# Parskatt/RoMa

Hardware: NVIDIA H100
Metric: image-pairs/sec match()+sample() 560->864 (higher is better)
Workload: dtype f32 (activations f32; GEMM operands as split-f16 pairs hi + 2^-11 lo on wgmma, f32 accumulate: fp32-class)

## Files before the change

### include/romab200.h

```cpp
#ifndef ROMAB200_H
#define ROMAB200_H

#include <stdint.h>

#ifdef __cplusplus
extern "C" {
#endif

#define ROMAB200_ABI_VERSION 4

enum rb_dtype { RB_F32 = 0, RB_F16 = 1, RB_BF16 = 2, RB_F16S = 3, RB_F64 = 4 };
enum rb_act { RB_ACT_NONE = 0, RB_ACT_RELU = 1, RB_ACT_GELU = 2 };
enum rb_rowmap { RB_ROWMAP_NONE = 0, RB_ROWMAP_PAD_KEEP = 1, RB_ROWMAP_PAD_TO_COMPACT = 2, RB_ROWMAP_SEGMENT = 3 };
enum rb_epi { RB_EPI_LINEAR = 0, RB_EPI_COSKERNEL = 1 };
enum rb_backend { RB_BACKEND_AUTO = 0, RB_BACKEND_SIMT = 1, RB_BACKEND_TCGEN05 = 2 };

int romab200_abi_version(void);
const char* romab200_last_error(void);
unsigned long long romab200_launch_count(void);
int romab200_device_ok(void);

typedef struct {
    const void* A; const void* B; void* C;
    int32_t M, N, K;
    int64_t lda, ldb, ldc;
    int32_t dtype_ab, dtype_c;
    int32_t trans_b;
    int32_t batch0, batch1;
    int64_t sa0, sa1, sb0, sb1, sc0, sc1;
    int32_t ntaps; int32_t tap_rows[9]; int64_t a_rows;
    float alpha;
    const float* bias; const float* col_scale;
    const void* R; int64_t ldr, sr0, sr1; int32_t dtype_r;
    int32_t act;
    int32_t epi;
    const float* norm_a; const float* norm_b; int64_t sna0, snb0;
    float eps, inv_t, diag_add; int32_t cos_normalized;
    int32_t rowmap, pad_h, pad_w, seg_in, seg_out, seg_off;
    int32_t backend;
    const void* A_lo; const void* B_lo; void* C_lo;
    int32_t max_ctas;
} rb_gemm_args;
int romab200_gemm(const rb_gemm_args* args, void* stream);

typedef struct {
    const void* x; void* y; const float* gamma; const float* beta;
    int64_t rows; int32_t cols; int64_t ldx, ldy; int32_t dtype_x, dtype_y; float eps;
    void* y_lo;
} rb_layernorm_args;
int romab200_layernorm(const rb_layernorm_args* args, void* stream);

typedef struct { void* s; int64_t rows; int32_t cols; int64_t lds; int32_t dtype; float scale;
                 void* out_hi; void* out_lo; int64_t ldo; } rb_softmax_args;
int romab200_softmax_rows(const rb_softmax_args* args, void* stream);

typedef struct {
    const void* qkv; void* out; int64_t ld_qkv, ld_out; int32_t batch, n_tokens, heads, head_dim, dtype;
    const void* qkv_lo; void* out_lo;
} rb_flash_attn_args;
int romab200_flash_attn(const rb_flash_attn_args* args, void* stream);

typedef struct { const void* x; float* out; int64_t rows; int32_t cols; int64_t ldx; int32_t dtype; } rb_rownorm_args;
int romab200_row_norms(const rb_rownorm_args* args, void* stream);

typedef struct {
    const void* src; void* dst; int64_t rows; int32_t cols; int64_t lds, ldd; int32_t dtype_src, dtype_dst;
    const float* row_scale; int32_t row_scale_reciprocal;
} rb_copy2d_args;
int romab200_copy2d(const rb_copy2d_args* args, void* stream);

typedef struct {
    const void* src; void* dst; const int32_t* src_index; const int32_t* dst_index;
    int32_t count; int64_t row_bytes, ld_src, ld_dst; int32_t src_rows, dst_rows;
} rb_gather_rows_args;
int romab200_gather_rows(const rb_gather_rows_args* args, void* stream);

typedef struct {
    const float* x; void* dst; int64_t rows; int32_t cols; int64_t ldx, ldd; const float* row_norm;
    int32_t layout_b;
} rb_split_args;
int romab200_split_f16x3(const rb_split_args* args, void* stream);

typedef struct {
    const float* x; void* hi; void* lo; int64_t rows; int32_t cols; int64_t ldx, ldd; const float* row_norm;
} rb_split_pair_args;
int romab200_split_f16s(const rb_split_pair_args* args, void* stream);

typedef struct {
    const float* image; void* out; const float* weight ; const float* bias ;
    int32_t batch, height, width, cout; int32_t dtype_out;
    void* out_lo;
} rb_conv_first_args;
int romab200_conv3x3_first(const rb_conv_first_args* args, void* stream);
typedef struct { const void* in; void* out; int32_t batch, height, width, channels, dtype;
                 const void* in_lo; void* out_lo;  } rb_maxpool_args;
int romab200_maxpool2x2_padded(const rb_maxpool_args* args, void* stream);

typedef struct { const float* image; void* out; int32_t batch, height, width, patch; int64_t ldo; int32_t dtype_out; } rb_im2col_args;
int romab200_im2col_patch(const rb_im2col_args* args, void* stream);
typedef struct { const float* patch; const float* cls; const float* pos; float* tokens; int32_t batch, npatch, dim; } rb_tokens_args;
int romab200_assemble_tokens(const rb_tokens_args* args, void* stream);

typedef struct {
    float* W; int32_t n, nrhs, batch; int64_t ldw, stride;
    void* workspace; int64_t workspace_bytes;
    int32_t algo;
} rb_gp_solve_args;
int romab200_gp_solve(const rb_gp_solve_args* args, void* stream);
typedef struct { const void* logits; float* state; int64_t rows; int64_t ldl; int32_t res; int32_t dtype; } rb_cls_args;
int romab200_cls_to_flow_refine(const rb_cls_args* args, void* stream);

typedef struct {
    const void* feat; int64_t ldf; int32_t n_img, y_shift;
    const float* state; void* d; int64_t ldd;
    int32_t D, h, w, cf, emb, radius; int32_t dtype;
    const float* emb_weight ; const float* emb_bias; float disp_scale;
    const float* grid_x; const float* grid_y;
    const float* win_x; const float* win_y;
    void* tile_done; int32_t tile_done_len;
    const float* corr_table; int64_t ld_corr_table;
} rb_refiner_prologue_args;
int romab200_refiner_prologue(const rb_refiner_prologue_args* args, void* stream);

typedef struct {
    const void* f0; const void* f1; int64_t ldf0, ldf1; int64_t f0_img_stride, f1_img_stride;
    const float* flow; int64_t ldflow; void* out; int64_t ldo;
    int32_t batch, h, w, c, radius; float scale; int32_t dtype_f, dtype_out;
    int32_t n_img, y_shift;
    const float* win_x; const float* win_y;
} rb_local_corr_args;
int romab200_local_corr(const rb_local_corr_args* args, void* stream);

typedef struct {
    const float* f0; const float* f1; int64_t ldf0, ldf1; const float* warp; float* out;
    int32_t batch, h, w, c, k; int32_t mode;
} rb_local_corr_warp_args;
int romab200_local_corr_warp(const rb_local_corr_warp_args* args, void* stream);

typedef struct {
    const void* in; void* out; int64_t ldi, ldo; const float* weight; int64_t ldw; const float* bias;
    int32_t batch, h, w, c; int32_t dtype;
    void* out_lo;
} rb_dwconv_args;
int romab200_dwconv5x5_relu(const rb_dwconv_args* args, void* stream);

typedef struct {
    const void* in; void* out; int64_t ld; const float* dw_weight; int64_t ldw; const float* dw_bias;
    const float* pw_weight_host; const float* pw_bias_host; int32_t batch, h, w, c; int32_t dtype;
} rb_refiner_block_small_args;
int romab200_refiner_block_small(const rb_refiner_block_small_args* args, void* stream);

typedef struct {
    const void* in; void* out; int64_t ld; const float* dw_weight; int64_t ldw; const float* dw_bias;
    const void* pw_weight; int64_t ld_pw; const float* pw_bias; int32_t batch, h, w, c; int32_t dtype;
} rb_refiner_block_c144_args;
int romab200_refiner_block_c144(const rb_refiner_block_c144_args* args, void* stream);

typedef struct {
    const float* in; float* out; int64_t ld; const float* dw_weight; int64_t ldw; const float* dw_bias;
    const void* pw_weight; const void* pw_weight_lo; int64_t ld_pw; const float* pw_bias; int32_t batch, h, w, c;
} rb_refiner_block_c144_split_args;
int romab200_refiner_block_c144_split(const rb_refiner_block_c144_split_args* args, void* stream);

typedef struct {
    const void* d; int64_t ldd; const float* weight ; int64_t ldw; const float* bias;
    float* state; int64_t rows; int32_t c; float scale_x, scale_y; int32_t dtype; float* delta_out ;
} rb_refiner_tail_args;
int romab200_refiner_tail(const rb_refiner_tail_args* args, void* stream);

typedef struct { const float* in; float* out; int32_t batch, hi, wi, ho, wo, c; } rb_resize_args;
int romab200_bilinear_resize(const rb_resize_args* args, void* stream);

typedef struct {
    const float* state; const float* coarse_state; int32_t hc, wc;
    float* warp; float* cert; int32_t b, H, W, symmetric;
    const float* grid_x; const float* grid_y;
} rb_match_epilogue_args;
int romab200_match_epilogue(const rb_match_epilogue_args* args, void* stream);

typedef struct { const float* x; float* density; int32_t n; float std; int32_t half;
                 float* workspace; int32_t splits;
                 int32_t symmetric; int64_t workspace_floats;
                 int32_t batch; } rb_kde_args;
int romab200_kde_density(const rb_kde_args* args, void* stream);

enum rb_sample_transform { RB_SAMPLE_IDENTITY = 0, RB_SAMPLE_THRESHOLD = 1, RB_SAMPLE_BALANCE = 2 };
typedef struct {
    const float* values; int64_t n; int32_t k; int32_t batch; int64_t stride; uint64_t seed; int32_t transform; float param;
    int32_t* out_idx; float* out_weights; float* keys;
    void* scratch;
    const uint64_t* seed_dev;
    int64_t seed_stride; int32_t repeats;
} rb_sample_args;
int romab200_weighted_sample(const rb_sample_args* args, void* stream);

typedef struct {
    const float* matches; const float* certainty; int64_t n;
    const int32_t* idx; int32_t items, k, repeats;
    int32_t threshold; float thresh;
    float* out_matches; float* out_certainty;
} rb_sample_gather_args;
int romab200_sample_gather(const rb_sample_gather_args* args, void* stream);

typedef struct { int32_t in_size, out_size; int32_t* bounds; int32_t* kk; int32_t* ksize; } rb_resample_coeffs_args;
int romab200_resample_coeffs(const rb_resample_coeffs_args* args, void* stream);

typedef struct {
    const uint8_t* in; int64_t ld_in ; int32_t in_h, in_w;
    int32_t out_h, out_w;
    const int32_t* bounds_x; const int32_t* kk_x; int32_t ksize_x;
    const int32_t* bounds_y; const int32_t* kk_y; int32_t ksize_y;
    uint8_t* tmp;
    uint8_t* out_u8;
    float* out;
    float mean[3]; float std[3];
} rb_preprocess_args;
int romab200_preprocess_rgb8(const rb_preprocess_args* args, void* stream);

typedef struct {
    const void* src; void* dst; int32_t rows, cols; int64_t lds, ldd; int32_t batch0, batch1;
    int64_t ss0, ss1, sd0, sd1; int32_t dtype;
} rb_transpose_args;
int romab200_transpose(const rb_transpose_args* args, void* stream);

typedef struct {
    const float* x; int32_t n;
    const float* warp; int32_t warp_h, warp_w; int64_t warp_ld_row, warp_ld_px, warp_ld_ch;
    const float* cert; int32_t cert_h, cert_w; int64_t cert_ld_row, cert_ld_px;
    float* x_to_B; float* cert_out;
} rb_keypoints_sample_args;
int romab200_keypoints_sample(const rb_keypoints_sample_args* args, void* stream);

typedef struct {
    const float* x_A_to_B; const float* cert_A; const float* x_B; int32_t n_a, n_b;
    float cert_th, max_dist;
    float* workspace; int64_t workspace_floats;
    int64_t* offsets;
    int64_t* inds_A; int64_t* inds_B;
} rb_keypoints_mnn_args;
int romab200_keypoints_mnn_count(const rb_keypoints_mnn_args* args, void* stream);
int romab200_keypoints_mnn_emit(const rb_keypoints_mnn_args* args, void* stream);

typedef struct {
    const float* in; float* out; const float* weight; const float* bias; const float* col_scale; const float* R;
    int64_t ldi, ldo, ldw, ldr;
    int32_t batch, hi, wi, ho, wo, cin, cout, ksize, stride, relu;
} rb_tiny_conv_args;
int romab200_tiny_conv(const rb_tiny_conv_args* args, void* stream);

typedef struct { const float* in; float* out; int32_t batch, channels, h, w, instance_norm; float eps; } rb_tiny_gray_args;
int romab200_tiny_gray(const rb_tiny_gray_args* args, void* stream);

typedef struct { const float* in; float* out; int32_t batch, hi, wi, c; } rb_tiny_avgpool_args;
int romab200_tiny_avgpool4(const rb_tiny_avgpool_args* args, void* stream);

typedef struct { const float* a; const float* b; const float* c; float* out; int64_t n; } rb_tiny_add3_args;
int romab200_tiny_add3(const rb_tiny_add3_args* args, void* stream);

typedef struct {
    const float* f0; const float* f1; float* state;
    int32_t batch, h0, w0, h1, w1, c; float scale; int32_t exact;
    const float* grid_x; const float* grid_y; const float* grid_lr_x; const float* grid_lr_y;
} rb_tiny_pos_embed_args;
int romab200_tiny_pos_embed(const rb_tiny_pos_embed_args* args, void* stream);

typedef struct {
    const float* f0; const float* f1; const float* state; float* out;
    int64_t ldf0, ldf1, lds, ldo; int32_t batch, h0, w0, h1, w1, c;
} rb_tiny_warp_concat_args;
int romab200_tiny_warp_concat(const rb_tiny_warp_concat_args* args, void* stream);

typedef struct { const float* state; float* warp; float* cert; int32_t batch, h, w; const float* grid_x; const float* grid_y; } rb_tiny_epilogue_args;
int romab200_tiny_match_epilogue(const rb_tiny_epilogue_args* args, void* stream);

typedef struct {
    int32_t batch;
    const uint8_t* stream;
    const int64_t* desc;
    const int32_t* tables;
    uint8_t* comp;
    int32_t* chunks;
    int32_t* istart;
    int64_t* exits;
    int32_t* counts;
    int16_t* coef;
    int32_t* state;
    int32_t* flags;
    int32_t max_chunks, max_intervals;
    int64_t total_slots, total_blocks;
    uint8_t* planes;
    uint8_t* out;
    int64_t max_pixels;
} rb_jpeg_args;
int romab200_jpeg_entropy(const rb_jpeg_args* args, void* stream);
int romab200_jpeg_pixels(const rb_jpeg_args* args, void* stream);

#define RB_POSE_ROUND 1024
#define RB_POSE_MAX_SOL 10
#define RB_POSE_MAX_SPLITS 16
#define RB_POSE_STATE 8
typedef struct {
    int32_t batch;
    const double* x0; const double* x1;
    const int64_t* offsets;
    const double* K;
    int64_t max_n;
    double thresh, conf;
    int32_t max_iters, round;
    uint64_t seed;
    double* xn;
    int32_t* sample;
    double* E;
    int32_t* nsol;
    int32_t* counts;
    int32_t* state;
    double* best_E;
    int32_t* running;
    double* R; double* t;
    uint8_t* ok;
    uint8_t* mask;
} rb_pose_args;
int romab200_pose_hypotheses(const rb_pose_args* args, void* stream);
int romab200_pose_score(const rb_pose_args* args, void* stream);
int romab200_pose_select(const rb_pose_args* args, void* stream);
int romab200_pose_recover(const rb_pose_args* args, void* stream);

#define RB_HOMOG_ROUND 2048
#define RB_HOMOG_MAX_SPLITS 32
#define RB_HOMOG_MAX_ATTEMPTS 10000
#define RB_HOMOG_STATE 8
typedef struct {
    int32_t batch;
    const float* src; const float* dst;
    const int64_t* offsets;
    int64_t max_n;
    double thresh, conf;
    int32_t max_iters, round, method;
    uint64_t seed;
    int32_t* sample;
    int32_t* attempts;
    int32_t* status;
    double* H;
    int32_t* counts;
    int32_t* state;
// ... 328 lines not shown
```

### roma_b200/csrc/gemm_tc.cu

```cuda
#include "tma.cuh"
#include "wgmma.cuh"

namespace rb {

struct TcParams {
    int M, N, K;
    int batch1;
    int ntaps, k_per_tap; int tap_rows[9];
    int tiles_m, tiles_n, total_tiles;
    int band_m;
    int n_zero_to;
    int64_t sc0, sc1, sr0, sr1, sna0, snb0;
    Epilogue epi;
};

constexpr int TC_BM = 128, TC_BK = 64;
constexpr int TC_THREADS = 384;
constexpr int TC_CW = 32, TC_SP = 40;
constexpr int TC_STAGING = 2 * 64 * TC_SP * 4;

template <int BN, bool SPLIT> struct TcCfg {
    static constexpr int NOPS = SPLIT ? 2 : 1;
    static constexpr int A_BYTES = TC_BM * TC_BK * 2;
    static constexpr int B_BYTES = BN * TC_BK * 2;
    static constexpr int STAGE_BYTES = NOPS * (A_BYTES + B_BYTES);
    static constexpr int RING_MAX = 232448 - TC_STAGING - 1024  - 256 ;
    static constexpr int STAGES = RING_MAX / STAGE_BYTES > 8 ? 8 : RING_MAX / STAGE_BYTES;
    static constexpr int SMEM = STAGES * STAGE_BYTES + TC_STAGING + 1024 + 256;
    static_assert(STAGES >= 3 && SMEM <= 232448, "shared memory budget");
};

__device__ __forceinline__ void load8(const void* p, int64_t i, int dtype, int cnt, float (&v)[8]) {
    if (dtype == RB_F32) {
        const float* s = (const float*)p + i;
        if (cnt == 8 && (reinterpret_cast<uintptr_t>(s) & 15) == 0) {
            const float4 a = reinterpret_cast<const float4*>(s)[0], b = reinterpret_cast<const float4*>(s)[1];
            v[0] = a.x; v[1] = a.y; v[2] = a.z; v[3] = a.w; v[4] = b.x; v[5] = b.y; v[6] = b.z; v[7] = b.w;
        } else {
#pragma unroll
            for (int k = 0; k < 8; ++k) v[k] = k < cnt ? s[k] : 0.f;
        }
        return;
    }
    const uint16_t* s = (const uint16_t*)p + i;
    uint16_t h[8];
    if (cnt == 8 && (reinterpret_cast<uintptr_t>(s) & 15) == 0) {
        const uint4 q = *reinterpret_cast<const uint4*>(s);
        const uint32_t w[4] = {q.x, q.y, q.z, q.w};
#pragma unroll
        for (int k = 0; k < 4; ++k) { h[2 * k] = (uint16_t)w[k]; h[2 * k + 1] = (uint16_t)(w[k] >> 16); }
    } else {
#pragma unroll
        for (int k = 0; k < 8; ++k) h[k] = k < cnt ? s[k] : 0;
    }
    if (dtype == RB_F16) {
#pragma unroll
        for (int k = 0; k < 8; ++k) v[k] = __half2float(__ushort_as_half(h[k]));
    } else {
#pragma unroll
        for (int k = 0; k < 8; ++k) v[k] = __bfloat162float(__ushort_as_bfloat16(h[k]));
    }
}

__device__ __forceinline__ void store8(const Epilogue& e, int64_t i, int cnt, const float (&v)[8]) {
    if (e.dtype_c == RB_F32) {
        float* c = (float*)e.C + i;
        if (cnt == 8 && (reinterpret_cast<uintptr_t>(c) & 15) == 0) {
            reinterpret_cast<float4*>(c)[0] = make_float4(v[0], v[1], v[2], v[3]);
            reinterpret_cast<float4*>(c)[1] = make_float4(v[4], v[5], v[6], v[7]);
        } else {
#pragma unroll
            for (int k = 0; k < 8; ++k) if (k < cnt) c[k] = v[k];
        }
        return;
    }
    uint16_t h[8], l[8];
    const bool two = e.dtype_c == RB_F16S;
    if (e.dtype_c == RB_BF16) {
#pragma unroll
        for (int k = 0; k < 8; ++k) h[k] = __bfloat16_as_ushort(__float2bfloat16_rn(v[k]));
    } else {
#pragma unroll
        for (int k = 0; k < 8; ++k) {
            __half hi, lo;
            split_f16s(v[k], hi, lo);
            h[k] = __half_as_ushort(hi); l[k] = __half_as_ushort(lo);
        }
    }
    uint16_t* c = (uint16_t*)e.C + i;
    uint16_t* cl = two ? (uint16_t*)e.C_lo + i : nullptr;
    if (cnt == 8 && (reinterpret_cast<uintptr_t>(c) & 15) == 0 && (!two || (reinterpret_cast<uintptr_t>(cl) & 15) == 0)) {
        *reinterpret_cast<uint4*>(c) = make_uint4(h[0] | (uint32_t)h[1] << 16, h[2] | (uint32_t)h[3] << 16, h[4] | (uint32_t)h[5] << 16,
                                                  h[6] | (uint32_t)h[7] << 16);
        if (two) *reinterpret_cast<uint4*>(cl) = make_uint4(l[0] | (uint32_t)l[1] << 16, l[2] | (uint32_t)l[3] << 16,
                                                            l[4] | (uint32_t)l[5] << 16, l[6] | (uint32_t)l[7] << 16);
    } else {
#pragma unroll
        for (int k = 0; k < 8; ++k) if (k < cnt) { c[k] = h[k]; if (two) cl[k] = l[k]; }
    }
}

__device__ __forceinline__ void epilogue8(const Epilogue& e, int m, int n, int64_t orow, int cnt, const float (&cb)[8],
                                          const float (&cs)[8], float na, float (&v)[8]) {
    const int nv = min(8, e.N - n);
    if (e.epi == RB_EPI_COSKERNEL) {
#pragma unroll
        for (int k = 0; k < 8; ++k) {
            const float p = na * cb[k];
            const float s = e.cos_normalized ? p / (p + e.eps) : 1.0f / (p + e.eps);
            v[k] = expf((v[k] * s - 1.0f) * e.inv_t);
            if (m == n + k) v[k] += e.diag_add;
        }
    } else {
#pragma unroll
        for (int k = 0; k < 8; ++k) v[k] = __fmul_rn(e.alpha, v[k]);
        if (e.bias) {
#pragma unroll
            for (int k = 0; k < 8; ++k) v[k] = __fadd_rn(v[k], cb[k]);
        }
        if (e.act == RB_ACT_RELU) {
#pragma unroll
            for (int k = 0; k < 8; ++k) v[k] = fmaxf(v[k], 0.0f);
        } else if (e.act == RB_ACT_GELU) {
#pragma unroll
            for (int k = 0; k < 8; ++k) v[k] = gelu_erf(v[k]);
        }
        if (e.col_scale) {
#pragma unroll
            for (int k = 0; k < 8; ++k) v[k] = __fmul_rn(v[k], cs[k]);
        }
        if (e.R) {
            float r[8];
            load8(e.R, orow * e.ldr + n, e.dtype_r, nv, r);
#pragma unroll
            for (int k = 0; k < 8; ++k) v[k] = __fadd_rn(v[k], r[k]);
        }
    }
    if (nv < 8) {
#pragma unroll
        for (int k = 0; k < 8; ++k) if (k >= nv) v[k] = 0.f;
    }
    store8(e, orow * e.ldc + n, cnt, v);
}

__device__ __forceinline__ void tile_coords(const TcParams& p, int w, int& z, int& mt, int& nt) {
    const int per_z = p.tiles_m * p.tiles_n;
    z = w / per_z;
    const int r = w - z * per_z;
    const int m_lo = r / (p.band_m * p.tiles_n) * p.band_m;
    const int rows = min(p.band_m, p.tiles_m - m_lo);
    const int rb = r - m_lo * p.tiles_n;
    nt = rb / rows;
    mt = m_lo + (rb - nt * rows);
}

template <int BN, bool SPLIT, bool BF16, int TB>
__global__ void __launch_bounds__(TC_THREADS, 1)
gemm_tc_kernel(const __grid_constant__ CUtensorMap map_a, const __grid_constant__ CUtensorMap map_b,
               const __grid_constant__ CUtensorMap map_a_lo, const __grid_constant__ CUtensorMap map_b_lo, const TcParams p) {
    using Cfg = TcCfg<BN, SPLIT>;
    constexpr int STAGES = Cfg::STAGES;
    constexpr int A_BYTES = Cfg::A_BYTES, B_BYTES = Cfg::B_BYTES;
    constexpr int OFF_A_LO = A_BYTES, OFF_B = Cfg::NOPS * A_BYTES, OFF_B_LO = Cfg::NOPS * A_BYTES + B_BYTES;
    extern __shared__ uint8_t smem_raw[];
    uint8_t* smem = smem_raw + ((1024u - ((uint32_t)__cvta_generic_to_shared(smem_raw) & 1023u)) & 1023u);
    float* staging = reinterpret_cast<float*>(smem + STAGES * Cfg::STAGE_BYTES);
    uint64_t* full_bar = reinterpret_cast<uint64_t*>(smem + STAGES * Cfg::STAGE_BYTES + TC_STAGING);
    uint64_t* empty_bar = full_bar + STAGES;

    const int warp = threadIdx.x >> 5, lane = threadIdx.x & 31;
    const int kblocks = (p.K + TC_BK - 1) / TC_BK;

    if (threadIdx.x == 0) {
        for (int s = 0; s < STAGES; ++s) { mbar_init(&full_bar[s], 1); mbar_init(&empty_bar[s], 2); }
        asm volatile("fence.mbarrier_init.release.cluster;" ::: "memory");
    }
    __syncthreads();
    rb::pdl_wait();

    if (warp >= 8) {
        asm volatile("setmaxnreg.dec.sync.aligned.u32 40;");
        if (warp == 8 && lane == 0) {
            const int kb_per_tap = p.ntaps > 1 ? p.k_per_tap / TC_BK : kblocks;
            uint32_t it = 0;
            for (int tile = blockIdx.x; tile < p.total_tiles; tile += gridDim.x) {
                int z, mt, nt;
                tile_coords(p, tile, z, mt, nt);
                const int m0 = mt * TC_BM, n0 = nt * BN, z0 = z / p.batch1, z1 = z - z0 * p.batch1;
                for (int kb = 0; kb < kblocks; ++kb, ++it) {
                    const int s = it % STAGES;
                    const uint32_t ph = (it / STAGES) & 1;
                    mbar_wait(&empty_bar[s], ph ^ 1);
                    mbar_expect_tx(&full_bar[s], Cfg::STAGE_BYTES);
                    int tap = 0, kin = kb * TC_BK, shift = 0;
                    if (p.ntaps > 1) { tap = kb / kb_per_tap; kin = (kb - tap * kb_per_tap) * TC_BK; shift = p.tap_rows[tap]; }
                    uint8_t* st = smem + s * Cfg::STAGE_BYTES;
                    tma_load_4d(st, &map_a, &full_bar[s], kin, m0 + shift, z1, z0);
                    if constexpr (SPLIT) tma_load_4d(st + OFF_A_LO, &map_a_lo, &full_bar[s], kin, m0 + shift, z1, z0);
                    if constexpr (!TB) {
                        tma_load_4d(st + OFF_B, &map_b, &full_bar[s], kb * TC_BK, n0, z1, z0);
                        if constexpr (SPLIT) tma_load_4d(st + OFF_B_LO, &map_b_lo, &full_bar[s], kb * TC_BK, n0, z1, z0);
                    } else {
#pragma unroll
                        for (int j = 0; j < (BN + 63) / 64; ++j) {
                            tma_load_4d(st + OFF_B + j * (64 * 128), &map_b, &full_bar[s], n0 + j * 64, kb * TC_BK, z1, z0);
                            if constexpr (SPLIT) tma_load_4d(st + OFF_B_LO + j * (64 * 128), &map_b_lo, &full_bar[s], n0 + j * 64, kb * TC_BK, z1, z0);
                        }
                    }
                }
            }
        }
        return;
    }

    asm volatile("setmaxnreg.inc.sync.aligned.u32 232;");
    const int wg = warp >> 2, t = threadIdx.x & 127;
    float acc[BN / 2];
    float acc2[SPLIT ? BN / 2 : 1];
    uint32_t it = 0;
    for (int tile = blockIdx.x; tile < p.total_tiles; tile += gridDim.x) {
        int z, mt, nt;
        tile_coords(p, tile, z, mt, nt);
        const int m0 = mt * TC_BM, n0 = nt * BN, z0 = z / p.batch1, z1 = z - z0 * p.batch1;
        int prev = -1;
        for (int kb = 0; kb < kblocks; ++kb, ++it) {
            const int s = it % STAGES;
            mbar_wait(&full_bar[s], (it / STAGES) & 1);
            const uint32_t st = smem_u32(smem + s * Cfg::STAGE_BYTES);
            wgmma_fence();
#pragma unroll
            for (int k = 0; k < TC_BK / 16; ++k) {
                const uint32_t koff_a = wg * (64 * 128) + k * 32;
                const uint32_t koff_b = TB ? k * 2048 : k * 32;
                const uint32_t lbo_b = TB ? 64 * 128 : 16;
                const uint64_t a_hi = gmma_desc(st + koff_a, 16, 1024);
                const uint64_t b_hi = gmma_desc(st + OFF_B + koff_b, lbo_b, 1024);
                const int accum = (kb | k) != 0;
                Wgmma<BN, BF16>::template ss<TB>(acc, a_hi, b_hi, accum);
                if constexpr (SPLIT) {
                    const uint64_t a_lo = gmma_desc(st + OFF_A_LO + koff_a, 16, 1024);
                    const uint64_t b_lo = gmma_desc(st + OFF_B_LO + koff_b, lbo_b, 1024);
                    Wgmma<BN, BF16>::template ss<TB>(acc2, a_hi, b_lo, accum);
                    Wgmma<BN, BF16>::template ss<TB>(acc2, a_lo, b_hi, 1);
                }
            }
            wgmma_commit();
            wgmma_wait<1>();
            if (prev >= 0 && t == 0) mbar_arrive(&empty_bar[prev]);
            prev = s;
        }
        wgmma_wait<0>();
        wgmma_fence_regs(acc);
        if constexpr (SPLIT) wgmma_fence_regs(acc2);
        if (t == 0) mbar_arrive(&empty_bar[prev]);

        Epilogue e = p.epi;
        e.C = (char*)e.C + (z0 * p.sc0 + z1 * p.sc1) * dtype_size(e.dtype_c);
        if (e.C_lo) e.C_lo = (char*)e.C_lo + (z0 * p.sc0 + z1 * p.sc1) * 2;
        if (e.R) e.R = (const char*)e.R + (z0 * p.sr0 + z1 * p.sr1) * dtype_size(e.dtype_r);
        if (e.norm_a) e.norm_a += z0 * p.sna0;
        if (e.norm_b) e.norm_b += z0 * p.snb0;
        float* stg = staging + wg * (64 * TC_SP);
        const int fr = (t >> 5) * 16 + ((t & 31) >> 2), fc = 2 * (t & 3);
        const int g = t & 3, rr = t >> 2;
        int mrow[2]; int64_t orow[2]; float na[2] = {0.f, 0.f};
#pragma unroll
        for (int h = 0; h < 2; ++h) {
            mrow[h] = m0 + wg * 64 + rr + 32 * h;
            orow[h] = mrow[h] < e.M ? e.map_row(mrow[h]) : -1;
            if (orow[h] >= 0 && e.epi == RB_EPI_COSKERNEL) na[h] = e.norm_a[mrow[h]];
        }
        constexpr int NCH = (BN + TC_CW - 1) / TC_CW;
#pragma unroll 1
        for (int ch = 0; ch < NCH; ++ch) {
            if (n0 + ch * TC_CW >= p.n_zero_to) break;
            bar_named(1 + wg, 128);
#pragma unroll
            for (int c = 0; c < NCH; ++c) {
                if (c != ch) continue;
#pragma unroll
                for (int jj = 0; jj < TC_CW / 8; ++jj) {
                    const int j = c * (TC_CW / 8) + jj;
                    if (j >= BN / 8) break;
#pragma unroll
                    for (int h = 0; h < 2; ++h) {
                        float v0 = acc[4 * j + 2 * h], v1 = acc[4 * j + 2 * h + 1];
                        if constexpr (SPLIT) {
                            v0 = fmaf(acc2[4 * j + 2 * h], 1.0f / RB_SPLIT_SCALE, v0);
                            v1 = fmaf(acc2[4 * j + 2 * h + 1], 1.0f / RB_SPLIT_SCALE, v1);
                        }
                        *reinterpret_cast<float2*>(stg + (fr + 8 * h) * TC_SP + 8 * jj + fc) = make_float2(v0, v1);
                    }
                }
            }
            bar_named(1 + wg, 128);
            const int n = n0 + ch * TC_CW + 8 * g;
            if (ch * TC_CW + 8 * g >= BN || n >= p.n_zero_to) continue;
            const int cnt = min(8, p.n_zero_to - n);
            float cb[8], cs[8];
            const float* colb = e.epi == RB_EPI_COSKERNEL ? e.norm_b : e.bias;
#pragma unroll
            for (int k = 0; k < 8; ++k) {
                const bool in = n + k < e.N;
                cb[k] = colb && in ? colb[n + k] : 0.f;
                cs[k] = e.col_scale && in ? e.col_scale[n + k] : 0.f;
            }
#pragma unroll
            for (int h = 0; h < 2; ++h) {
                if (orow[h] < 0) continue;
                const float* src = stg + (rr + 32 * h) * TC_SP + 8 * g;
                const int q = (rr & 1) * 4;
                const float4 a = *reinterpret_cast<const float4*>(src + q), b = *reinterpret_cast<const float4*>(src + (4 - q));
                float v[8];
                if (q == 0) { v[0] = a.x; v[1] = a.y; v[2] = a.z; v[3] = a.w; v[4] = b.x; v[5] = b.y; v[6] = b.z; v[7] = b.w; }
                else        { v[0] = b.x; v[1] = b.y; v[2] = b.z; v[3] = b.w; v[4] = a.x; v[5] = a.y; v[6] = a.z; v[7] = a.w; }
                epilogue8(e, mrow[h], n, orow[h], cnt, cb, cs, na[h], v);
            }
        }
    }
}

static int make_map(CUtensorMap* map, const void* base, int dtype, uint64_t inner, uint64_t rows, uint64_t pitch_elems, uint64_t b1,
                    uint64_t s1_elems, uint64_t b0, uint64_t s0_elems, uint32_t box_inner, uint32_t box_rows) {
    RB_REQUIRE(((uintptr_t)base) % 16 == 0 && (pitch_elems * 2) % 16 == 0, "gemm_tc: operand base/pitch must be 16-byte aligned (pitch %llu elems)", (unsigned long long)pitch_elems);
    RB_REQUIRE((b1 <= 1 || (s1_elems * 2) % 16 == 0) && (b0 <= 1 || (s0_elems * 2) % 16 == 0), "gemm_tc: batch strides must be 16-byte aligned");
    cuuint64_t dims[4] = {inner, rows, b1 > 0 ? b1 : 1, b0 > 0 ? b0 : 1};
    cuuint64_t strides[3] = {pitch_elems * 2, (b1 > 1 ? s1_elems : pitch_elems * rows) * 2, (b0 > 1 ? s0_elems : pitch_elems * rows) * 2};
    cuuint32_t box[4] = {box_inner, box_rows, 1, 1};
    return encode_tiled(map, "gemm_tc", tma_dtype(dtype), 4, base, dims, strides, box,
                        CU_TENSOR_MAP_SWIZZLE_128B);
}

struct TcMaps { CUtensorMap a, b, a_lo, b_lo; };

template <int BN, bool SPLIT, bool BF16, int TB>
static int launch_tc(const TcMaps& maps, TcParams& p, int zdim, int max_ctas, cudaStream_t st) {
    using Cfg = TcCfg<BN, SPLIT>;
    auto kernel = gemm_tc_kernel<BN, SPLIT, BF16, TB>;
    if (ensure_smem<gemm_tc_kernel<BN, SPLIT, BF16, TB>>(Cfg::SMEM, "gemm_tc")) return 1;
    p.tiles_m = (p.M + TC_BM - 1) / TC_BM;
    p.tiles_n = (p.N + BN - 1) / BN;
    const long long total = (long long)p.tiles_m * p.tiles_n * zdim;
    RB_REQUIRE(total < (1ll << 31), "gemm_tc: too many tiles");
    p.total_tiles = (int)total;
    int resident = sm_count();
    if (max_ctas > 0 && max_ctas < resident) resident = max_ctas;
    const int grid = p.total_tiles < resident ? p.total_tiles : resident;
    const int64_t a_bytes = (int64_t)p.M * (p.ntaps > 1 ? p.k_per_tap : p.K) * Cfg::NOPS * 2;
    const int64_t b_bytes = (int64_t)p.N * p.K * Cfg::NOPS * 2;
    const bool bands = p.tiles_n > 1 && 2 * a_bytes > l2_bytes() && 2 * b_bytes <= l2_bytes();
    const int band_m = grid / p.tiles_n > 1 ? grid / p.tiles_n : 1;
    p.band_m = bands && band_m < p.tiles_m ? band_m : p.tiles_m;
    cudaError_t err = rb::launch_pdl(kernel, dim3(grid), dim3(TC_THREADS), Cfg::SMEM, st, maps.a, maps.b, maps.a_lo, maps.b_lo, (const TcParams)p);
    if (err != cudaSuccess) { set_error("gemm_tc: launch failed: %s", cudaGetErrorString(err)); return 1; }
    return check_launch("gemm_tc");
}

template <bool SPLIT, bool BF16>
static int dispatch_tc(int BN, int trans_b, const TcMaps& maps, TcParams& p, int zdim, int max_ctas, cudaStream_t st) {
    if (trans_b) return BN == 64 ? launch_tc<64, SPLIT, BF16, 1>(maps, p, zdim, max_ctas, st) : launch_tc<128, SPLIT, BF16, 1>(maps, p, zdim, max_ctas, st);
    switch (BN) {
        case 32: return launch_tc<32, SPLIT, BF16, 0>(maps, p, zdim, max_ctas, st);
        case 64: return launch_tc<64, SPLIT, BF16, 0>(maps, p, zdim, max_ctas, st);
        case 128: return launch_tc<128, SPLIT, BF16, 0>(maps, p, zdim, max_ctas, st);
        case 144: return launch_tc<144, SPLIT, BF16, 0>(maps, p, zdim, max_ctas, st);
        default:
            if constexpr (SPLIT) { set_error("gemm_tc: split-fp16 tiles are at most 144 columns wide (got %d)", BN); return 1; }
            else {
                switch (BN) {
                    case 192: return launch_tc<192, false, BF16, 0>(maps, p, zdim, max_ctas, st);
                    default: return launch_tc<256, false, BF16, 0>(maps, p, zdim, max_ctas, st);
                }
            }
    }
}

int gemm_tc(const rb_gemm_args* a, cudaStream_t stream) {
    RB_REQUIRE(a->dtype_ab == RB_F16 || a->dtype_ab == RB_BF16 || a->dtype_ab == RB_F16S, "gemm_tc: operands must be fp16/bf16/split-fp16 (got %d)", a->dtype_ab);
    RB_REQUIRE(a->M > 0 && a->N > 0 && a->K > 0, "gemm_tc: empty problem");
    const bool split = a->dtype_ab == RB_F16S;
    RB_REQUIRE(!split || (a->A_lo && a->B_lo), "gemm_tc: split-fp16 operands need A_lo and B_lo");
    RB_REQUIRE(a->dtype_c != RB_F16S || a->C_lo, "gemm_tc: split-fp16 output needs C_lo");
    TcParams p;
    p.M = a->M; p.N = a->N; p.K = a->K;
    p.batch1 = a->batch1 > 0 ? a->batch1 : 1;
    const int batch0 = a->batch0 > 0 ? a->batch0 : 1;
    p.ntaps = a->ntaps > 1 ? a->ntaps : 1;
    p.k_per_tap = a->K / p.ntaps;
    for (int i = 0; i < 9; ++i) p.tap_rows[i] = a->tap_rows[i];
    const bool bf16 = a->dtype_ab == RB_BF16;
    p.sc0 = a->sc0; p.sc1 = a->sc1; p.sr0 = a->sr0; p.sr1 = a->sr1; p.sna0 = a->sna0; p.snb0 = a->snb0;
    p.epi = make_epilogue(a);
    if (p.ntaps > 1) {
        RB_REQUIRE(a->K % p.ntaps == 0 && p.k_per_tap % TC_BK == 0, "gemm_tc: K/ntaps=%d must be a multiple of %d", p.k_per_tap, TC_BK);
        RB_REQUIRE(!a->trans_b && batch0 * p.batch1 == 1, "gemm_tc: taps need un-batched [N,K] weights");
    }
    const int zdim = batch0 * p.batch1;
    RB_REQUIRE(zdim <= 65535, "gemm_tc: batch too large");
    const int64_t a_rows = a->a_rows > 0 ? a->a_rows : a->M;
    int BN = a->N <= 32 && !a->trans_b ? 32 : (a->N <= 64 ? 64 : 128);
    if (!a->trans_b && a->N > 128) {
        if (split) BN = (a->N + 143) / 144 * 144 < (a->N + 127) / 128 * 128 ? 144 : 128;
        else if (a->N <= 144) BN = 144;
        else if (a->N <= 192) BN = 192;
        else {
            const int w192 = (a->N + 191) / 192 * 192 - a->N, w256 = (a->N + 255) / 256 * 256 - a->N;
            BN = (w192 + a->N / 20 < w256) ? 192 : 256;
        }
        if (((int64_t)((a->M + 127) / 128) * ((a->N + BN - 1) / BN) * zdim) < sm_count() * 2 / 3) BN = 128;
    }
    TcMaps maps;
    const uint64_t a_inner = p.ntaps > 1 ? p.k_per_tap : a->K;
    if (make_map(&maps.a, a->A, a->dtype_ab, a_inner, a_rows, a->lda, p.batch1, a->sa1, batch0, a->sa0, TC_BK, TC_BM)) return 1;
    if (split && make_map(&maps.a_lo, a->A_lo, a->dtype_ab, a_inner, a_rows, a->lda, p.batch1, a->sa1, batch0, a->sa0, TC_BK, TC_BM)) return 1;
    if (!a->trans_b) {
        if (make_map(&maps.b, a->B, a->dtype_ab, a->K, a->N, a->ldb, p.batch1, a->sb1, batch0, a->sb0, TC_BK, BN)) return 1;
        if (split && make_map(&maps.b_lo, a->B_lo, a->dtype_ab, a->K, a->N, a->ldb, p.batch1, a->sb1, batch0, a->sb0, TC_BK, BN)) return 1;
    } else {
        if (make_map(&maps.b, a->B, a->dtype_ab, a->N, a->K, a->ldb, p.batch1, a->sb1, batch0, a->sb0, 64, TC_BK)) return 1;
        if (split && make_map(&maps.b_lo, a->B_lo, a->dtype_ab, a->N, a->K, a->ldb, p.batch1, a->sb1, batch0, a->sb0, 64, TC_BK)) return 1;
    }
    if (!split) { maps.a_lo = maps.a; maps.b_lo = maps.b; }
    {
        const int es_c = dtype_size(a->dtype_c);
        const bool align_ok = ((uintptr_t)a->C) % 16 == 0 && (a->ldc * es_c) % 16 == 0 && (p.batch1 <= 1 || (a->sc1 * es_c) % 16 == 0) &&
                              (batch0 <= 1 || (a->sc0 * es_c) % 16 == 0) && (a->dtype_c != RB_F16S || ((uintptr_t)a->C_lo) % 16 == 0);
        const bool rowmap_ok = a->rowmap == RB_ROWMAP_NONE || a->rowmap == RB_ROWMAP_PAD_KEEP;
        const int gran = 16 / es_c;
        p.n_zero_to = align_ok && rowmap_ok && !a->R ? (a->N + gran - 1) / gran * gran : a->N;
    }
    if (split) return dispatch_tc<true, false>(BN, a->trans_b, maps, p, zdim, a->max_ctas, stream);
    return bf16 ? dispatch_tc<false, true>(BN, a->trans_b, maps, p, zdim, a->max_ctas, stream)
                : dispatch_tc<false, false>(BN, a->trans_b, maps, p, zdim, a->max_ctas, stream);
}

}
```

### roma_b200/csrc/tma.cuh

```cuda
#pragma once
#include "common.cuh"
#include <cuda.h>
#include <cudaTypedefs.h>

namespace rb {

__device__ __forceinline__ uint32_t smem_u32(const void* p) { return (uint32_t)__cvta_generic_to_shared(p); }

__device__ __forceinline__ void mbar_init(uint64_t* bar, uint32_t count) {
    asm volatile("mbarrier.init.shared::cta.b64 [%0], %1;" ::"r"(smem_u32(bar)), "r"(count));
}
__device__ __forceinline__ void mbar_expect_tx(uint64_t* bar, uint32_t bytes) {
    asm volatile("mbarrier.arrive.expect_tx.shared::cta.b64 _, [%0], %1;" ::"r"(smem_u32(bar)), "r"(bytes) : "memory");
}
__device__ __forceinline__ void mbar_arrive(uint64_t* bar) {
    asm volatile("mbarrier.arrive.shared::cta.b64 _, [%0];" ::"r"(smem_u32(bar)) : "memory");
}
__device__ __forceinline__ void mbar_wait(uint64_t* bar, uint32_t parity) {
    const uint32_t addr = smem_u32(bar);
    uint32_t done;
    do {
        asm volatile(
            "{\n"
            ".reg .pred p;\n"
            "mbarrier.try_wait.parity.shared::cta.b64 p, [%1], %2;\n"
            "selp.u32 %0, 1, 0, p;\n"
            "}\n" : "=r"(done) : "r"(addr), "r"(parity) : "memory");
    } while (!done);
}
__device__ __forceinline__ void tma_load_2d(void* smem_dst, const CUtensorMap* map, uint64_t* bar, int c0, int c1) {
    asm volatile(
        "cp.async.bulk.tensor.2d.shared::cluster.global.mbarrier::complete_tx::bytes [%0], [%1, {%3, %4}], [%2];"
        ::"r"(smem_u32(smem_dst)), "l"(reinterpret_cast<uint64_t>(map)), "r"(smem_u32(bar)), "r"(c0), "r"(c1)
        : "memory");
}
__device__ __forceinline__ void tma_load_3d(void* smem_dst, const CUtensorMap* map, uint64_t* bar, int c0, int c1, int c2) {
    asm volatile(
        "cp.async.bulk.tensor.3d.shared::cluster.global.mbarrier::complete_tx::bytes [%0], [%1, {%3, %4, %5}], [%2];"
        ::"r"(smem_u32(smem_dst)), "l"(reinterpret_cast<uint64_t>(map)), "r"(smem_u32(bar)), "r"(c0), "r"(c1), "r"(c2)
        : "memory");
}
__device__ __forceinline__ void tma_load_4d(void* smem_dst, const CUtensorMap* map, uint64_t* bar, int c0, int c1, int c2, int c3) {
    asm volatile(
        "cp.async.bulk.tensor.4d.shared::cluster.global.mbarrier::complete_tx::bytes [%0], [%1, {%3, %4, %5, %6}], [%2];"
        ::"r"(smem_u32(smem_dst)), "l"(reinterpret_cast<uint64_t>(map)), "r"(smem_u32(bar)), "r"(c0), "r"(c1), "r"(c2), "r"(c3)
        : "memory");
}

__device__ __forceinline__ void bar_named(int id, int nthreads) { asm volatile("bar.sync %0, %1;" ::"r"(id), "r"(nthreads) : "memory"); }
__device__ __forceinline__ void bar_arrive(int id, int nthreads) { asm volatile("bar.arrive %0, %1;" ::"r"(id), "r"(nthreads) : "memory"); }

inline PFN_cuTensorMapEncodeTiled_v12000 tensor_map_encoder() {
    static const PFN_cuTensorMapEncodeTiled_v12000 fn = [] {
        void* ptr = nullptr;
        cudaDriverEntryPointQueryResult q;
        const bool ok = cudaGetDriverEntryPoint("cuTensorMapEncodeTiled", &ptr, cudaEnableDefault, &q) == cudaSuccess && ptr;
        return ok ? reinterpret_cast<PFN_cuTensorMapEncodeTiled_v12000>(ptr) : nullptr;
    }();
    return fn;
}

inline CUtensorMapDataType tma_dtype(int code) {
    return code == RB_F32 ? CU_TENSOR_MAP_DATA_TYPE_FLOAT32 : (code == RB_BF16 ? CU_TENSOR_MAP_DATA_TYPE_BFLOAT16 : CU_TENSOR_MAP_DATA_TYPE_FLOAT16);
}

inline int encode_tiled(CUtensorMap* map, const char* what, CUtensorMapDataType dtype, int rank, const void* base, const cuuint64_t* dims,
                        const cuuint64_t* strides, const cuuint32_t* box, CUtensorMapSwizzle swizzle) {
    const PFN_cuTensorMapEncodeTiled_v12000 enc = tensor_map_encoder();
    RB_REQUIRE(enc, "%s: cuTensorMapEncodeTiled not available (driver too old?)", what);
    const cuuint32_t estr[5] = {1, 1, 1, 1, 1};
    const CUresult r = enc(map, dtype, (cuuint32_t)rank, const_cast<void*>(base), dims, strides, box, estr, CU_TENSOR_MAP_INTERLEAVE_NONE,
                           swizzle, CU_TENSOR_MAP_L2_PROMOTION_L2_256B, CU_TENSOR_MAP_FLOAT_OOB_FILL_NONE);
    RB_REQUIRE(r == CUDA_SUCCESS, "%s: cuTensorMapEncodeTiled failed with %d (dims %llu x %llu x ..., pitch %llu bytes)", what, (int)r,
               (unsigned long long)dims[0], (unsigned long long)dims[1], (unsigned long long)strides[0]);
    return 0;
}

template <auto Kernel>
inline int ensure_smem(int bytes, const char* what) {
    static bool configured[64] = {};
    const int dev = current_device() & 63;
    if (!configured[dev]) {
        const cudaError_t e = cudaFuncSetAttribute(Kernel, cudaFuncAttributeMaxDynamicSharedMemorySize, bytes);
        RB_REQUIRE(e == cudaSuccess, "%s: cannot set %d bytes of dynamic shared memory: %s", what, bytes, cudaGetErrorString(e));
        configured[dev] = true;
    }
    return 0;
}

inline int sm_count() {
    static int n[64] = {};
    const int dev = current_device() & 63;
    if (!n[dev]) {
        cudaDeviceGetAttribute(&n[dev], cudaDevAttrMultiProcessorCount, dev);
        if (n[dev] <= 0) n[dev] = 132;
    }
    return n[dev];
}

inline int64_t l2_bytes() {
    static int n[64] = {};
    const int dev = current_device() & 63;
    if (!n[dev]) {
        cudaDeviceGetAttribute(&n[dev], cudaDevAttrL2CacheSize, dev);
        if (n[dev] <= 0) n[dev] = 50 << 20;
    }
    return n[dev];
}

}
```

Before: 17.73.

## Add thread-block cluster TMA multicast to split-fp16 GEMM kernel

Adds optional 2x1/1x2/2x2 thread-block clusters to the split-f16 wgmma GEMM. Each CTA loads a slice of the shared A or B tile and multicasts it to its cluster peers. Stage release becomes a cross-CTA mbarrier arrive to every peer that wrote into the stage. Auto mode picks 2x1 only for banded, L2-pressured single-tap shapes, to cut global/L2 traffic for the shared operand. The cost is cluster synchronisation overhead, coarser tile scheduling that can leave tiles idle, and reliance on occupancy queries for clusters.

```diff
diff --git a/include/romab200.h b/include/romab200.h
--- a/include/romab200.h
+++ b/include/romab200.h
@@ -40,6 +40,7 @@
     int32_t backend;
     const void* A_lo; const void* B_lo; void* C_lo;
     int32_t max_ctas;
+    int32_t cluster;
 } rb_gemm_args;
 int romab200_gemm(const rb_gemm_args* args, void* stream);
 
diff --git a/roma_b200/csrc/gemm_tc.cu b/roma_b200/csrc/gemm_tc.cu
--- a/roma_b200/csrc/gemm_tc.cu
+++ b/roma_b200/csrc/gemm_tc.cu
@@ -154,7 +154,7 @@
     mt = m_lo + (rb - nt * rows);
 }
 
-template <int BN, bool SPLIT, bool BF16, int TB>
+template <int BN, bool SPLIT, bool BF16, int TB, int CM = 1, int CN = 1>
 __global__ void __launch_bounds__(TC_THREADS, 1)
 gemm_tc_kernel(const __grid_constant__ CUtensorMap map_a, const __grid_constant__ CUtensorMap map_b,
                const __grid_constant__ CUtensorMap map_a_lo, const __grid_constant__ CUtensorMap map_b_lo, const TcParams p) {
@@ -162,6 +162,8 @@
     constexpr int STAGES = Cfg::STAGES;
     constexpr int A_BYTES = Cfg::A_BYTES, B_BYTES = Cfg::B_BYTES;
     constexpr int OFF_A_LO = A_BYTES, OFF_B = Cfg::NOPS * A_BYTES, OFF_B_LO = Cfg::NOPS * A_BYTES + B_BYTES;
+    constexpr int CS = CM * CN;
+    static_assert(CS == 1 || (SPLIT && !TB), "clusters serve the split-fp16 kernel with [N, K] B");
     extern __shared__ uint8_t smem_raw[];
     uint8_t* smem = smem_raw + ((1024u - ((uint32_t)__cvta_generic_to_shared(smem_raw) & 1023u)) & 1023u);
     float* staging = reinterpret_cast<float*>(smem + STAGES * Cfg::STAGE_BYTES);
@@ -170,22 +172,32 @@
 
     const int warp = threadIdx.x >> 5, lane = threadIdx.x & 31;
     const int kblocks = (p.K + TC_BK - 1) / TC_BK;
+    const int rank = blockIdx.x % CS, rx = rank % CM, ry = rank / CM;
+    const int work0 = blockIdx.x / CS, work_step = gridDim.x / CS;
 
     if (threadIdx.x == 0) {
-        for (int s = 0; s < STAGES; ++s) { mbar_init(&full_bar[s], 1); mbar_init(&empty_bar[s], 2); }
+        for (int s = 0; s < STAGES; ++s) { mbar_init(&full_bar[s], 1); mbar_init(&empty_bar[s], 2 * (CM + CN - 1)); }
         asm volatile("fence.mbarrier_init.release.cluster;" ::: "memory");
     }
-    __syncthreads();
+    if constexpr (CS > 1) cluster_sync();
+    else __syncthreads();
     rb::pdl_wait();
 
     if (warp >= 8) {
         asm volatile("setmaxnreg.dec.sync.aligned.u32 40;");
         if (warp == 8 && lane == 0) {
             const int kb_per_tap = p.ntaps > 1 ? p.k_per_tap / TC_BK : kblocks;
+            uint16_t mask_a = 0, mask_b = 0;
+#pragma unroll
+            for (int j = 0; j < CN; ++j) mask_a |= (uint16_t)(1u << (rx + CM * j));
+#pragma unroll
+            for (int i = 0; i < CM; ++i) mask_b |= (uint16_t)(1u << (i + CM * ry));
+            constexpr int A_ROWS = TC_BM / CN, B_ROWS = BN / CM;
             uint32_t it = 0;
-            for (int tile = blockIdx.x; tile < p.total_tiles; tile += gridDim.x) {
+            for (int tile = work0; tile < p.total_tiles; tile += work_step) {
                 int z, mt, nt;
                 tile_coords(p, tile, z, mt, nt);
+                if constexpr (CS > 1) { mt = mt * CM + rx; nt = nt * CN + ry; }
                 const int m0 = mt * TC_BM, n0 = nt * BN, z0 = z / p.batch1, z1 = z - z0 * p.batch1;
                 for (int kb = 0; kb < kblocks; ++kb, ++it) {
                     const int s = it % STAGES;
@@ -195,6 +207,24 @@
                     int tap = 0, kin = kb * TC_BK, shift = 0;
                     if (p.ntaps > 1) { tap = kb / kb_per_tap; kin = (kb - tap * kb_per_tap) * TC_BK; shift = p.tap_rows[tap]; }
                     uint8_t* st = smem + s * Cfg::STAGE_BYTES;
+                    if constexpr (CS > 1) {
+                        const int ra = ry * A_ROWS, rb = rx * B_ROWS;
+                        if constexpr (CN > 1) {
+                            tma_load_4d_mc(st + ra * 128, &map_a, &full_bar[s], mask_a, kin, m0 + shift + ra, z1, z0);
+                            tma_load_4d_mc(st + OFF_A_LO + ra * 128, &map_a_lo, &full_bar[s], mask_a, kin, m0 + shift + ra, z1, z0);
+                        } else {
+                            tma_load_4d(st, &map_a, &full_bar[s], kin, m0 + shift, z1, z0);
+                            tma_load_4d(st + OFF_A_LO, &map_a_lo, &full_bar[s], kin, m0 + shift, z1, z0);
+                        }
+                        if constexpr (CM > 1) {
+                            tma_load_4d_mc(st + OFF_B + rb * 128, &map_b, &full_bar[s], mask_b, kb * TC_BK, n0 + rb, z1, z0);
+                            tma_load_4d_mc(st + OFF_B_LO + rb * 128, &map_b_lo, &full_bar[s], mask_b, kb * TC_BK, n0 + rb, z1, z0);
+                        } else {
+                            tma_load_4d(st + OFF_B, &map_b, &full_bar[s], kb * TC_BK, n0, z1, z0);
+                            tma_load_4d(st + OFF_B_LO, &map_b_lo, &full_bar[s], kb * TC_BK, n0, z1, z0);
+                        }
+                        continue;
+                    }
                     tma_load_4d(st, &map_a, &full_bar[s], kin, m0 + shift, z1, z0);
                     if constexpr (SPLIT) tma_load_4d(st + OFF_A_LO, &map_a_lo, &full_bar[s], kin, m0 + shift, z1, z0);
                     if constexpr (!TB) {
@@ -210,17 +240,24 @@
                 }
             }
         }
+        if constexpr (CS > 1) cluster_sync();
         return;
     }
 
     asm volatile("setmaxnreg.inc.sync.aligned.u32 232;");
     const int wg = warp >> 2, t = threadIdx.x & 127;
+    int release_rank = rank;
+    if constexpr (CS > 1) {
+        if (t >= 1 && t < CN) release_rank = rx + CM * ((ry + t) % CN);
+        else if (t >= CN) release_rank = (rx + t - CN + 1) % CM + CM * ry;
+    }
     float acc[BN / 2];
     float acc2[SPLIT ? BN / 2 : 1];
     uint32_t it = 0;
-    for (int tile = blockIdx.x; tile < p.total_tiles; tile += gridDim.x) {
+    for (int tile = work0; tile < p.total_tiles; tile += work_step) {
         int z, mt, nt;
         tile_coords(p, tile, z, mt, nt);
+        if constexpr (CS > 1) { mt = mt * CM + rx; nt = nt * CN + ry; }
         const int m0 = mt * TC_BM, n0 = nt * BN, z0 = z / p.batch1, z1 = z - z0 * p.batch1;
         int prev = -1;
         for (int kb = 0; kb < kblocks; ++kb, ++it) {
@@ -246,13 +283,17 @@
             }
             wgmma_commit();
             wgmma_wait<1>();
-            if (prev >= 0 && t == 0) mbar_arrive(&empty_bar[prev]);
+            if (prev >= 0) {
+                if constexpr (CS > 1) { if (t < CM + CN - 1) mbar_arrive_cluster(&empty_bar[prev], release_rank); }
+                else if (t == 0) mbar_arrive(&empty_bar[prev]);
+            }
             prev = s;
         }
         wgmma_wait<0>();
         wgmma_fence_regs(acc);
         if constexpr (SPLIT) wgmma_fence_regs(acc2);
-        if (t == 0) mbar_arrive(&empty_bar[prev]);
+        if constexpr (CS > 1) { if (t < CM + CN - 1) mbar_arrive_cluster(&empty_bar[prev], release_rank); }
+        else if (t == 0) mbar_arrive(&empty_bar[prev]);
 
         Epilogue e = p.epi;
         e.C = (char*)e.C + (z0 * p.sc0 + z1 * p.sc1) * dtype_size(e.dtype_c);
@@ -318,6 +359,7 @@
             }
         }
     }
+    if constexpr (CS > 1) cluster_sync();
 }
 
 static int make_map(CUtensorMap* map, const void* base, int dtype, uint64_t inner, uint64_t rows, uint64_t pitch_elems, uint64_t b1,
@@ -333,32 +375,88 @@
 
 struct TcMaps { CUtensorMap a, b, a_lo, b_lo; };
 
-template <int BN, bool SPLIT, bool BF16, int TB>
+template <auto Kernel, int CS, int SMEM>
+static int max_active_clusters() {
+    static int n[64] = {};
+    const int dev = current_device() & 63;
+    if (!n[dev]) {
+        cudaLaunchConfig_t cfg = {};
+        cfg.gridDim = dim3(CS * sm_count()); cfg.blockDim = dim3(TC_THREADS); cfg.dynamicSmemBytes = SMEM;
+        cudaLaunchAttribute attr[1];
+        attr[0].id = cudaLaunchAttributeClusterDimension;
+        attr[0].val.clusterDim.x = CS; attr[0].val.clusterDim.y = 1; attr[0].val.clusterDim.z = 1;
+        cfg.attrs = attr; cfg.numAttrs = 1;
+        int c = 0;
+        if (cudaOccupancyMaxActiveClusters(&c, Kernel, &cfg) != cudaSuccess || c <= 0) { cudaGetLastError(); c = -1; }
+        n[dev] = c;
+    }
+    return n[dev];
+}
+
+template <int BN, bool SPLIT, bool BF16, int TB, int CM = 1, int CN = 1>
 static int launch_tc(const TcMaps& maps, TcParams& p, int zdim, int max_ctas, cudaStream_t st) {
     using Cfg = TcCfg<BN, SPLIT>;
-    auto kernel = gemm_tc_kernel<BN, SPLIT, BF16, TB>;
-    if (ensure_smem<gemm_tc_kernel<BN, SPLIT, BF16, TB>>(Cfg::SMEM, "gemm_tc")) return 1;
-    p.tiles_m = (p.M + TC_BM - 1) / TC_BM;
-    p.tiles_n = (p.N + BN - 1) / BN;
+    constexpr int CS = CM * CN;
+    auto kernel = gemm_tc_kernel<BN, SPLIT, BF16, TB, CM, CN>;
+    if (ensure_smem<gemm_tc_kernel<BN, SPLIT, BF16, TB, CM, CN>>(Cfg::SMEM, "gemm_tc")) return 1;
+    p.tiles_m = ((p.M + TC_BM - 1) / TC_BM + CM - 1) / CM;
+    p.tiles_n = ((p.N + BN - 1) / BN + CN - 1) / CN;
     const long long total = (long long)p.tiles_m * p.tiles_n * zdim;
     RB_REQUIRE(total < (1ll << 31), "gemm_tc: too many tiles");
     p.total_tiles = (int)total;
     int resident = sm_count();
-    if (max_ctas > 0 && max_ctas < resident) resident = max_ctas;
+    if constexpr (CS > 1) {
+        resident = max_active_clusters<gemm_tc_kernel<BN, SPLIT, BF16, TB, CM, CN>, CS, Cfg::SMEM>();
+        RB_REQUIRE(resident > 0, "gemm_tc: no %d-CTA cluster fits on the device", CS);
+    }
+    if (max_ctas > 0 && max_ctas / CS < resident) resident = max_ctas / CS;
+    RB_REQUIRE(resident > 0, "gemm_tc: max_ctas = %d is below the cluster size %d", max_ctas, CS);
     const int grid = p.total_tiles < resident ? p.total_tiles : resident;
     const int64_t a_bytes = (int64_t)p.M * (p.ntaps > 1 ? p.k_per_tap : p.K) * Cfg::NOPS * 2;
     const int64_t b_bytes = (int64_t)p.N * p.K * Cfg::NOPS * 2;
     const bool bands = p.tiles_n > 1 && 2 * a_bytes > l2_bytes() && 2 * b_bytes <= l2_bytes();
     const int band_m = grid / p.tiles_n > 1 ? grid / p.tiles_n : 1;
     p.band_m = bands && band_m < p.tiles_m ? band_m : p.tiles_m;
-    cudaError_t err = rb::launch_pdl(kernel, dim3(grid), dim3(TC_THREADS), Cfg::SMEM, st, maps.a, maps.b, maps.a_lo, maps.b_lo, (const TcParams)p);
+    cudaError_t err;
+    if constexpr (CS == 1) {
+        err = rb::launch_pdl(kernel, dim3(grid), dim3(TC_THREADS), Cfg::SMEM, st, maps.a, maps.b, maps.a_lo, maps.b_lo, (const TcParams)p);
+    } else {
+        cudaLaunchConfig_t cfg = {};
+        cfg.gridDim = dim3(grid * CS); cfg.blockDim = dim3(TC_THREADS); cfg.dynamicSmemBytes = Cfg::SMEM; cfg.stream = st;
+        cudaLaunchAttribute attr[2];
+        attr[0].id = cudaLaunchAttributeClusterDimension;
+        attr[0].val.clusterDim.x = CS; attr[0].val.clusterDim.y = 1; attr[0].val.clusterDim.z = 1;
+        attr[1].id = cudaLaunchAttributeProgrammaticStreamSerialization;
+        attr[1].val.programmaticStreamSerializationAllowed = 1;
+        cfg.attrs = attr; cfg.numAttrs = pdl_mode() ? 1 : 2;
+        err = cudaLaunchKernelEx(&cfg, kernel, maps.a, maps.b, maps.a_lo, maps.b_lo, (const TcParams)p);
+    }
     if (err != cudaSuccess) { set_error("gemm_tc: launch failed: %s", cudaGetErrorString(err)); return 1; }
     return check_launch("gemm_tc");
 }
 
+enum { TC_CLUSTER_AUTO = 0, TC_CLUSTER_NONE = 1, TC_CLUSTER_2x1 = 2, TC_CLUSTER_1x2 = 3, TC_CLUSTER_2x2 = 4 };
+
 template <bool SPLIT, bool BF16>
-static int dispatch_tc(int BN, int trans_b, const TcMaps& maps, TcParams& p, int zdim, int max_ctas, cudaStream_t st) {
+static int dispatch_tc(int BN, int trans_b, int cluster, const TcMaps& maps, TcParams& p, int zdim, int max_ctas, cudaStream_t st) {
     if (trans_b) return BN == 64 ? launch_tc<64, SPLIT, BF16, 1>(maps, p, zdim, max_ctas, st) : launch_tc<128, SPLIT, BF16, 1>(maps, p, zdim, max_ctas, st);
+    if constexpr (SPLIT) {
+        if (cluster != TC_CLUSTER_NONE) {
+#define RB_TC_CLUSTER(bn) \
+            switch (cluster) { \
+                case TC_CLUSTER_2x1: return launch_tc<bn, true, false, 0, 2, 1>(maps, p, zdim, max_ctas, st); \
+                case TC_CLUSTER_1x2: return launch_tc<bn, true, false, 0, 1, 2>(maps, p, zdim, max_ctas, st); \
+                default: return launch_tc<bn, true, false, 0, 2, 2>(maps, p, zdim, max_ctas, st); \
+            }
+            switch (BN) {
+                case 32: RB_TC_CLUSTER(32)
+                case 64: RB_TC_CLUSTER(64)
+                case 128: RB_TC_CLUSTER(128)
+                default: RB_TC_CLUSTER(144)
+            }
+#undef RB_TC_CLUSTER
+        }
+    }
     switch (BN) {
         case 32: return launch_tc<32, SPLIT, BF16, 0>(maps, p, zdim, max_ctas, st);
         case 64: return launch_tc<64, SPLIT, BF16, 0>(maps, p, zdim, max_ctas, st);
@@ -409,13 +507,27 @@
         }
         if (((int64_t)((a->M + 127) / 128) * ((a->N + BN - 1) / BN) * zdim) < sm_count() * 2 / 3) BN = 128;
     }
+    RB_REQUIRE(a->cluster >= TC_CLUSTER_AUTO && a->cluster <= TC_CLUSTER_2x2, "gemm_tc: cluster must be 0..4 (got %d)", a->cluster);
+    int cluster = TC_CLUSTER_NONE;
+    if (split && !a->trans_b) {
+        const int tm = (a->M + TC_BM - 1) / TC_BM, tn = (a->N + BN - 1) / BN;
+        cluster = a->cluster;
+        if (cluster == TC_CLUSTER_AUTO) {
+            const int64_t a_b = (int64_t)a->M * (p.ntaps > 1 ? p.k_per_tap : a->K) * 4, b_b = (int64_t)a->N * a->K * 4;
+            const bool banded = tn > 1 && 2 * a_b > l2_bytes() && 2 * b_b <= l2_bytes();
+            cluster = banded && p.ntaps == 1 && tm >= 2 ? TC_CLUSTER_2x1 : TC_CLUSTER_NONE;
+        }
+        if (a->max_ctas > 0 && a->max_ctas < (cluster == TC_CLUSTER_2x2 ? 4 : 2)) cluster = TC_CLUSTER_NONE;
+    }
+    const int cm = cluster == TC_CLUSTER_2x1 || cluster == TC_CLUSTER_2x2 ? 2 : 1;
+    const int cn = cluster == TC_CLUSTER_1x2 || cluster == TC_CLUSTER_2x2 ? 2 : 1;
     TcMaps maps;
     const uint64_t a_inner = p.ntaps > 1 ? p.k_per_tap : a->K;
-    if (make_map(&maps.a, a->A, a->dtype_ab, a_inner, a_rows, a->lda, p.batch1, a->sa1, batch0, a->sa0, TC_BK, TC_BM)) return 1;
-    if (split && make_map(&maps.a_lo, a->A_lo, a->dtype_ab, a_inner, a_rows, a->lda, p.batch1, a->sa1, batch0, a->sa0, TC_BK, TC_BM)) return 1;
+    if (make_map(&maps.a, a->A, a->dtype_ab, a_inner, a_rows, a->lda, p.batch1, a->sa1, batch0, a->sa0, TC_BK, TC_BM / cn)) return 1;
+    if (split && make_map(&maps.a_lo, a->A_lo, a->dtype_ab, a_inner, a_rows, a->lda, p.batch1, a->sa1, batch0, a->sa0, TC_BK, TC_BM / cn)) return 1;
     if (!a->trans_b) {
-        if (make_map(&maps.b, a->B, a->dtype_ab, a->K, a->N, a->ldb, p.batch1, a->sb1, batch0, a->sb0, TC_BK, BN)) return 1;
-        if (split && make_map(&maps.b_lo, a->B_lo, a->dtype_ab, a->K, a->N, a->ldb, p.batch1, a->sb1, batch0, a->sb0, TC_BK, BN)) return 1;
+        if (make_map(&maps.b, a->B, a->dtype_ab, a->K, a->N, a->ldb, p.batch1, a->sb1, batch0, a->sb0, TC_BK, BN / cm)) return 1;
+        if (split && make_map(&maps.b_lo, a->B_lo, a->dtype_ab, a->K, a->N, a->ldb, p.batch1, a->sb1, batch0, a->sb0, TC_BK, BN / cm)) return 1;
     } else {
         if (make_map(&maps.b, a->B, a->dtype_ab, a->N, a->K, a->ldb, p.batch1, a->sb1, batch0, a->sb0, 64, TC_BK)) return 1;
         if (split && make_map(&maps.b_lo, a->B_lo, a->dtype_ab, a->N, a->K, a->ldb, p.batch1, a->sb1, batch0, a->sb0, 64, TC_BK)) return 1;
@@ -429,9 +541,9 @@
         const int gran = 16 / es_c;
         p.n_zero_to = align_ok && rowmap_ok && !a->R ? (a->N + gran - 1) / gran * gran : a->N;
     }
-    if (split) return dispatch_tc<true, false>(BN, a->trans_b, maps, p, zdim, a->max_ctas, stream);
-    return bf16 ? dispatch_tc<false, true>(BN, a->trans_b, maps, p, zdim, a->max_ctas, stream)
-                : dispatch_tc<false, false>(BN, a->trans_b, maps, p, zdim, a->max_ctas, stream);
-}
-
-}
+    if (split) return dispatch_tc<true, false>(BN, a->trans_b, cluster, maps, p, zdim, a->max_ctas, stream);
+    return bf16 ? dispatch_tc<false, true>(BN, a->trans_b, cluster, maps, p, zdim, a->max_ctas, stream)
+                : dispatch_tc<false, false>(BN, a->trans_b, cluster, maps, p, zdim, a->max_ctas, stream);
+}
+
+}
diff --git a/roma_b200/csrc/tma.cuh b/roma_b200/csrc/tma.cuh
--- a/roma_b200/csrc/tma.cuh
+++ b/roma_b200/csrc/tma.cuh
@@ -45,6 +45,32 @@
         "cp.async.bulk.tensor.4d.shared::cluster.global.mbarrier::complete_tx::bytes [%0], [%1, {%3, %4, %5, %6}], [%2];"
         ::"r"(smem_u32(smem_dst)), "l"(reinterpret_cast<uint64_t>(map)), "r"(smem_u32(bar)), "r"(c0), "r"(c1), "r"(c2), "r"(c3)
         : "memory");
+}
+
+__device__ __forceinline__ void tma_load_4d_mc(void* smem_dst, const CUtensorMap* map, uint64_t* bar, uint16_t cta_mask, int c0, int c1,
+                                               int c2, int c3) {
+    asm volatile(
+        "cp.async.bulk.tensor.4d.shared::cluster.global.mbarrier::complete_tx::bytes.multicast::cluster"
+        " [%0], [%1, {%4, %5, %6, %7}], [%2], %3;"
+        ::"r"(smem_u32(smem_dst)), "l"(reinterpret_cast<uint64_t>(map)), "r"(smem_u32(bar)), "h"(cta_mask), "r"(c0), "r"(c1), "r"(c2),
+          "r"(c3)
+        : "memory");
+}
+__device__ __forceinline__ uint32_t cluster_ctarank() {
+    uint32_t r;
+    asm volatile("mov.u32 %0, %%cluster_ctarank;" : "=r"(r));
+    return r;
+}
+__device__ __forceinline__ void mbar_arrive_cluster(uint64_t* bar, uint32_t rank) {
+    asm volatile(
+        "{\n"
+        ".reg .b32 remote;\n"
+        "mapa.shared::cluster.u32 remote, %0, %1;\n"
+        "mbarrier.arrive.shared::cluster.b64 _, [remote];\n"
+        "}\n" ::"r"(smem_u32(bar)), "r"(rank) : "memory");
+}
+__device__ __forceinline__ void cluster_sync() {
+    asm volatile("barrier.cluster.arrive.release;\nbarrier.cluster.wait.acquire;" ::: "memory");
 }
 
 __device__ __forceinline__ void bar_named(int id, int nthreads) { asm volatile("bar.sync %0, %1;" ::"r"(id), "r"(nthreads) : "memory"); }
```

Measured after the change: 18.02 (median of 6 runs). 1.02x the previous value.
